# rkansal47/MPGAN

Measured on AMD Instinct MI355X. Metric: jets/sec (G+D step) MPGAN gluon N=30 bs=256 @1/2/4/8 MI355X, higher is better.
Workload: dtype split-16-bit MFMA, fp32 accumulate, fp32 in/out: f16 hi/lo x3 terms (forward), f16 x2 / x1 terms in per-sender dithered units (edge backward: data / weight gradients), bf16 hi/lo x3 (node network gradients); 1 GPU; MPGAN gluon-like jets (--jets g: lr_disc 3e-05, lr_gen 1e-05), N=30 particles, B=256 per GPU, one train_D+train_G iteration (LSGAN, RMSprop, D dropout 0.5); jets=g, loss=ls, fwd_two_term=False, global_batch=256, particles=30, multiplicity=gluon, parallelism=dp1, hip_graphs=True, graph_collectives=False

## Files before the change

include/mpgan_amd.h:

```cpp
#ifndef MPGAN_AMD_H
#define MPGAN_AMD_H
#include <stdint.h>
#ifdef __cplusplus
extern "C" {
#endif

typedef struct MpgGemm {
    const float* A;
    const float* A2;
    int lda, lda2, K1;
    const float* B;
    int ldb;
    float* C;
    int ldc;
    int M, N, K;
    long long split_stride;
    const float* bias;
    float out_scale;
    int act;
    float alpha;
    const uint64_t* seed;
    uint32_t drop_tag, drop_thr; float drop_scale;
    const float* gateH;
    int ldh, gate_act;
// ... 200 lines not shown
} MpgAttnDD;
int mpg_attn_dd(const MpgAttnDD* p, void* stream);

int mpg_rank_mask(const float* x, int ld_jet, int ld_part, const float* labels, int ld_lab, int B, int N,
                  float* mask, float* ignore, void* stream);

int mpg_jet_order(const float* mask, int B, int N, int* order, void* stream);

int mpg_gen_tail_fwd(const float* y, int ldy, const float* mask, float* out, int ldo, int V, int F, int act, void* stream);
int mpg_gen_tail_bwd(const float* dout, int ldd, const float* out, int ldo, float* dy, int ldy, int V, int F, int act,
                     void* stream);

typedef struct MpgDiscHead {
    const float* y; int ldy;
    const float* mask;
    const float* w; const float* bias;
    int B, N, F;
    int mean;
    int sigmoid;
    const uint64_t* seed; uint32_t tag, thr; float dscale;
    float* out;
    float* pooled; float* aux;
    int loss, gen_step, n_real; float inv_count;
    const float* gout;
    float* terms; float* loss_out;
    float* dy; int ld_dy;
    float* dw; float* db; int accumulate;
    const float* targets;
    const float* loss_extra;
} MpgDiscHead;
int mpg_disc_head_fwd(const MpgDiscHead* p, void* stream);
int mpg_disc_head_bwd(const MpgDiscHead* p, void* stream);
int mpg_disc_head_loss(const MpgDiscHead* p, void* stream);

typedef struct MpgDiscHeadDD {
    const float* y; int ldy;
    const float* mask;
    const float* w; const float* bias;
    int B, N, F, mean, sigmoid;
    const uint64_t* seed; uint32_t tag, thr; float dscale;
    int mode;
    const float* g;
    const float* U; int ldu;
    const float* mu;
    float* gy; int ld_gy;
    float* gm;
    float* gg;
    float* part;
    float* gw; float* gb;
} MpgDiscHeadDD;
int mpg_disc_head_dd(const MpgDiscHeadDD* p, void* stream);

typedef struct MpgBridge {
    const float* x; int ldx;
    const float* W1; const float* b1;
    int act1;
    float* feat; int ldf;
    int M, row0, K, F, E;
    const float* W2; const float* b2;
    int act2; float alpha;
    const uint64_t* seed; uint32_t tag, thr; float dscale;
    float* e; int lde;
} MpgBridge;
typedef struct MpgBridgeBwd {
    const float* ge; int ldge;
    const float* e; int lde;
// ... 191 lines not shown
```

mpgan_amd/_lib.py:

```python
from __future__ import annotations

import ctypes as C
import glob
import os
import subprocess

_HERE = os.path.dirname(os.path.abspath(__file__))
CSRC = os.path.join(_HERE, "csrc")
LIBDIR = os.environ.get("MPG_LIBDIR") or os.path.join(_HERE, "lib")
LIBPATH = os.path.join(LIBDIR, "libmpgan_amd.so")
INCLUDE = os.path.join(os.path.dirname(_HERE), "include")

_u64p = C.POINTER(C.c_uint64)
_fp = C.c_void_p


class MpgGemm(C.Structure):
    _fields_ = [
        ("A", _fp), ("A2", _fp), ("lda", C.c_int), ("lda2", C.c_int), ("K1", C.c_int),
        ("B", _fp), ("ldb", C.c_int),
        ("C", _fp), ("ldc", C.c_int),
        ("M", C.c_int), ("N", C.c_int), ("K", C.c_int),
        ("split_stride", C.c_longlong),
        ("bias", _fp), ("out_scale", C.c_float), ("act", C.c_int), ("alpha", C.c_float),
# ... 260 lines not shown
    "mpg_gemm_wgrad_group": (C.c_int, [C.POINTER(MpgGemm), C.POINTER(C.c_int), C.c_int, C.c_void_p]),
    "mpg_splitk_reduce_group": (C.c_int, [C.POINTER(MpgReduceJob), C.c_int, C.c_void_p]),
    "mpg_splitk_reduce_group_dw": (C.c_int, [C.POINTER(MpgReduceJob), C.c_int, C.POINTER(MpgEdgeDw), C.c_void_p]),
    "mpg_slab_sums": (C.c_int, [_fp, C.c_int, C.c_uint64, _fp, C.c_int, C.c_uint64, _fp, C.c_int, C.c_int, C.c_void_p]),
    "mpg_gate": (C.c_int, [_fp, C.c_int, _fp, C.c_int, _fp, C.c_int, C.c_int, C.c_int, C.c_int, C.c_float,
                           _fp, C.c_uint32, C.c_uint32, C.c_float, C.c_void_p]),
    "mpg_dropout_mask": (C.c_int, [_fp, C.c_uint64, C.c_int, _fp, C.c_uint32, C.c_uint32, C.c_void_p]),
    "mpg_pack_weights": (C.c_int, [_fp, C.c_int, C.c_int, C.c_int, C.c_int, C.c_float, C.c_int, _fp, C.c_void_p]),
    "mpg_pack_many": (C.c_int, [C.POINTER(MpgPackJob), C.c_int, C.c_void_p]),
    "mpg_chain": (C.c_int, [C.POINTER(MpgChain), C.c_void_p]),
    "mpg_chain_route": (C.c_int, [C.POINTER(MpgChain)]),
    "mpg_edge_fwd": (C.c_int, [C.POINTER(MpgEdgeFwd), C.c_void_p]),
    "mpg_edge_fwd_fn": (C.c_int, [C.POINTER(MpgEdgeFwd), C.POINTER(MpgChain), C.POINTER(MpgChain), C.c_void_p]),
    "mpg_edge_bwd": (C.c_int, [C.POINTER(MpgEdgeBwd), C.c_void_p]),
    "mpg_edge_bwd_fn": (C.c_int, [C.POINTER(MpgEdgeBwd), C.POINTER(MpgChain), C.POINTER(MpgChain), C.c_void_p]),
    "mpg_edge_dw": (C.c_int, [C.POINTER(MpgEdgeDw), C.c_void_p]),
    "mpg_attn_fwd": (C.c_int, [C.POINTER(MpgAttn), C.c_void_p]),
    "mpg_attn_bwd": (C.c_int, [C.POINTER(MpgAttn), C.c_void_p]),
    "mpg_attn_dd": (C.c_int, [C.POINTER(MpgAttnDD), C.c_void_p]),
    "mpg_mab_fwd": (C.c_int, [C.POINTER(MpgMab), C.c_void_p]),
    "mpg_mab_bwd": (C.c_int, [C.POINTER(MpgMab), C.c_void_p]),
    "mpg_mab_chain_fwd": (C.c_int, [C.POINTER(MpgMabChain), C.c_void_p]),
    "mpg_knn_edge_fwd": (C.c_int, [C.POINTER(MpgKnnEdgeFwd), C.c_void_p]),
    "mpg_knn_edge_bwd": (C.c_int, [C.POINTER(MpgKnnEdgeBwd), C.c_void_p]),
    "mpg_knn_edge_jvp": (C.c_int, [C.POINTER(MpgKnnEdgeJvp), C.c_void_p]),
    "mpg_knn_sets": (C.c_int, [_fp, C.c_int, _fp, C.c_int, C.c_int, C.c_int, C.c_int, C.c_int, _fp, C.c_void_p]),
    "mpg_rank_mask": (C.c_int, [_fp, C.c_int, C.c_int, _fp, C.c_int, C.c_int, C.c_int, _fp, _fp, C.c_void_p]),
    "mpg_jet_order": (C.c_int, [_fp, C.c_int, C.c_int, _fp, C.c_void_p]),
    "mpg_gen_tail_fwd": (C.c_int, [_fp, C.c_int, _fp, _fp, C.c_int, C.c_int, C.c_int, C.c_int, C.c_void_p]),
    "mpg_gen_tail_bwd": (C.c_int, [_fp, C.c_int, _fp, C.c_int, _fp, C.c_int, C.c_int, C.c_int, C.c_int, C.c_void_p]),
    "mpg_disc_head_fwd": (C.c_int, [C.POINTER(MpgDiscHead), C.c_void_p]),
    "mpg_disc_head_bwd": (C.c_int, [C.POINTER(MpgDiscHead), C.c_void_p]),
    "mpg_disc_head_loss": (C.c_int, [C.POINTER(MpgDiscHead), C.c_void_p]),
    "mpg_disc_head_dd": (C.c_int, [C.POINTER(MpgDiscHeadDD), C.c_void_p]),
    "mpg_layernorm_fwd": (C.c_int, [_fp, C.c_int, _fp, _fp, _fp, C.c_int, _fp, C.c_int, C.c_int, C.c_float, C.c_void_p]),
    "mpg_layernorm_bwd": (C.c_int, [_fp, C.c_int, _fp, C.c_int, _fp, _fp, _fp, C.c_int, _fp, C.c_int, _fp, _fp, C.c_int,
                                    C.c_int, C.c_int, C.c_void_p]),
    "mpg_batchnorm_stats": (C.c_int, [_fp, C.c_int, C.c_int, C.c_int, _fp, C.c_int, _fp, _fp, C.c_void_p]),
    "mpg_batchnorm_apply": (C.c_int, [_fp, C.c_int, _fp, _fp, _fp, _fp, C.c_float, _fp, C.c_int, C.c_int, C.c_int, C.c_void_p]),
    "mpg_batchnorm_bwd": (C.c_int, [_fp, C.c_int, _fp, C.c_int, _fp, _fp, _fp, C.c_float, _fp, C.c_int, _fp, _fp, C.c_int, _fp, _fp,
                                    C.c_int, C.c_int, C.c_int, C.c_void_p]),
    "mpg_rmsprop": (C.c_int, [_fp, _fp, _fp, C.c_uint64, C.c_float, C.c_float, C.c_float, C.c_float, C.c_int, _fp, C.c_uint64, C.c_void_p]),
    "mpg_adam": (C.c_int, [_fp, _fp, _fp, _fp, _fp, C.c_uint64, C.c_float, C.c_float, C.c_float, C.c_float, C.c_float,
                           C.c_float, C.c_int, _fp, C.c_uint64, C.c_void_p]),
    "mpg_adadelta": (C.c_int, [_fp, _fp, _fp, _fp, C.c_uint64, C.c_float, C.c_float, C.c_float, C.c_float, C.c_int, _fp, C.c_uint64,
                               C.c_void_p]),
    "mpg_rmsprop_ema": (C.c_int, [_fp, _fp, _fp, C.c_uint64, C.c_float, C.c_float, C.c_float, C.c_float, C.c_int, _fp, C.c_uint64,
                                  C.POINTER(MpgEma), C.c_void_p]),
    "mpg_adam_ema": (C.c_int, [_fp, _fp, _fp, _fp, _fp, C.c_uint64, C.c_float, C.c_float, C.c_float, C.c_float, C.c_float,
                               C.c_float, C.c_int, _fp, C.c_uint64, C.POINTER(MpgEma), C.c_void_p]),
    "mpg_adadelta_ema": (C.c_int, [_fp, _fp, _fp, _fp, C.c_uint64, C.c_float, C.c_float, C.c_float, C.c_float, C.c_int, _fp, C.c_uint64,
                                   C.POINTER(MpgEma), C.c_void_p]),
    "mpg_ema_update_host": (C.c_int, [_fp, _fp, C.c_uint64, C.c_uint32, C.c_float, C.c_int, C.c_int]),
    "mpg_step_control": (C.c_int, [_fp, C.c_uint64, C.c_float, C.POINTER(MpgStepCtl), C.c_void_p]),
    "mpg_step_control_host": (C.c_int, [_fp, C.c_uint64, C.c_float, C.POINTER(MpgStepCtl)]),
    "mpg_rmsprop_ctl": (C.c_int, [_fp, _fp, _fp, C.c_uint64, C.c_float, C.c_float, C.c_float, C.c_float, C.c_int, _fp, C.c_uint64,
                                  C.POINTER(MpgStepCtl), C.POINTER(MpgEma), C.c_void_p]),
    "mpg_adam_ctl": (C.c_int, [_fp, _fp, _fp, _fp, _fp, C.c_uint64, C.c_float, C.c_float, C.c_float, C.c_float, C.c_float,
                               C.c_float, C.c_int, _fp, C.c_uint64, C.POINTER(MpgStepCtl), C.POINTER(MpgEma), C.c_void_p]),
    "mpg_adadelta_ctl": (C.c_int, [_fp, _fp, _fp, _fp, C.c_uint64, C.c_float, C.c_float, C.c_float, C.c_float, C.c_int, _fp, C.c_uint64,
                                   C.POINTER(MpgStepCtl), C.POINTER(MpgEma), C.c_void_p]),
    "mpg_bridge_fwd": (C.c_int, [C.POINTER(MpgBridge), C.c_void_p]),
    "mpg_bridge_bwd": (C.c_int, [C.POINTER(MpgBridgeBwd), C.c_void_p]),
    "mpg_normal": (C.c_int, [_fp, C.c_uint64, _fp, C.c_uint32, C.c_float, C.c_float, C.c_void_p]),
    "mpg_normal_rank_mask": (C.c_int, [_fp, C.c_int, C.c_int, C.c_int, _fp, C.c_uint32, C.c_float, C.c_float, _fp, C.c_int, _fp, _fp,
                                       C.c_void_p]),
# ... 213 lines not shown
```

mpgan_amd/csrc/head.hip:

```cpp
#include "common.h"
#include "../../include/mpgan_amd.h"

namespace {

__global__ __launch_bounds__(256) void rank_mask_kernel(const float* __restrict__ x, int ld_jet, int ld_part,
                                                        const float* __restrict__ labels, int ld_lab, int N,
                                                        float* __restrict__ mask, float* __restrict__ ignore) {
    extern __shared__ float xs[];
    const int b = blockIdx.x;
    for (int i = threadIdx.x; i < N; i += blockDim.x) xs[i] = x[(size_t)b * ld_jet + (size_t)i * ld_part];
    __syncthreads();
    const int n_minus_1 = (int)(labels[(size_t)b * ld_lab] * (float)N) - 1;
    for (int i = threadIdx.x; i < N; i += blockDim.x) {
        const float xi = xs[i];
        int rank = 0;
        for (int j = 0; j < N; ++j) {
            const float xj = xs[j];
            rank += (xj < xi) || (xj == xi && j < i);
        }
        mask[(size_t)b * N + i] = rank <= n_minus_1 ? 1.f : 0.f;
        if (ignore != nullptr) ignore[(size_t)b * N + i] = rank <= n_minus_1 ? 0.f : 1.f;
    }
}

__global__ __launch_bounds__(1024) void jet_order_kernel(const float* __restrict__ mask, int B, int N, int* __restrict__ order) {
    extern __shared__ int jo[];
    int* keys = jo;
    int* hist = jo + B;
    int* wcnt = jo + B + N + 2;
    const int nw = (B + 63) / 64, lane = threadIdx.x & 63;
    for (int t = threadIdx.x; t < N + 2; t += blockDim.x) hist[t] = 0;
    for (int t = threadIdx.x; t < nw * (N + 1); t += blockDim.x) wcnt[t] = 0;
    __syncthreads();
// ... 18 lines not shown
    for (int b0 = (threadIdx.x >> 6) * 64; b0 < B; b0 += blockDim.x) {
        const int b = b0 + lane;
        const int k = b < B ? keys[b] : -1;
        int below = 0;
        for (int l = 0; l < 64; ++l) {
            const int kl = __shfl(k, l, 64);
            below += (l < lane && kl == k);
        }
        if (b < B) order[hist[k] + wcnt[(b >> 6) * (N + 1) + k] + below] = b;
    }
}

__global__ __launch_bounds__(256) void gen_tail_fwd_kernel(const float* __restrict__ y, int ldy, const float* __restrict__ mask,
                                                           float* __restrict__ out, int ldo, int V, int F, int act) {
    const int v = blockIdx.x * blockDim.x + threadIdx.x;
    if (v >= V) return;
    for (int f = 0; f < F; ++f) {
        const float t = y[(size_t)v * ldy + f];
        out[(size_t)v * ldo + f] = act == 1 ? tanhf(t) : (act == 2 ? 1.f / (1.f + expf(-t)) : t);
    }
    if (mask != nullptr) out[(size_t)v * ldo + F] = mask[v] - 0.5f;
}

__global__ __launch_bounds__(256) void gen_tail_bwd_kernel(const float* __restrict__ dout, int ldd, const float* __restrict__ out, int ldo,
                                                           float* __restrict__ dy, int ldy, int V, int F, int act) {
    const int v = blockIdx.x * blockDim.x + threadIdx.x;
    if (v >= V) return;
    for (int f = 0; f < F; ++f) {
        const float o = out[(size_t)v * ldo + f], g = dout[(size_t)v * ldd + f];
        dy[(size_t)v * ldy + f] = act == 1 ? g * (1.f - o * o) : (act == 2 ? g * o * (1.f - o) : g);
    }
}

MPG_DEV float wave_sum(float x) {
#pragma unroll
    for (int o = 32; o > 0; o >>= 1) x += __shfl_xor(x, o, 64);
    return x;
}

MPG_DEV void disc_head_bwd_jet(const MpgDiscHead& p, const int b, const int lane, const float out, const float aux0);

template <bool FUSED>
__global__ __launch_bounds__(256) void disc_head_fwd_kernel(const MpgDiscHead p) {
    const int lane = threadIdx.x & 63, b = blockIdx.x * 4 + (threadIdx.x >> 6);
    if (b >= p.B) return;
    const float* yb = p.y + (size_t)b * p.N * p.ldy;
    float z = 0.f, msum = 0.f;
    for (int f0 = 0; f0 < p.F; f0 += 32) {
        const int f = f0 + (lane & 31);
        float a0 = 0.f, a1 = 0.f, a2 = 0.f, a3 = 0.f;
        auto term = [&](int i) {
            return i < p.N ? (p.mask ? p.mask[(size_t)b * p.N + i] : 1.f) * yb[(size_t)i * p.ldy + f] : 0.f;
        };
        if (f < p.F)
            for (int i = lane >> 5; i < p.N; i += 8) { a0 += term(i); a1 += term(i + 2); a2 += term(i + 4); a3 += term(i + 6); }
        float acc = (a0 + a1) + (a2 + a3);
        acc += __shfl_xor(acc, 32, 64);
        if (p.pooled != nullptr && lane < 32 && f < p.F) p.pooled[(size_t)b * p.F + f] = acc;
        z += (lane < 32 && f < p.F) ? acc * p.w[f] : 0.f;
    }
    if (p.mean) {
        for (int i = lane; i < p.N; i += 64) msum += p.mask ? p.mask[(size_t)b * p.N + i] : 1.f;
        msum = wave_sum(msum);
    }
    z = wave_sum(z);
    const float pool_scale = p.mean ? 1.f / (p.mask ? msum + 1e-12f : (float)p.N) : 1.f;
    z = z * pool_scale + (p.bias ? p.bias[0] : 0.f);
    float keep = 1.f;
    if (p.thr) {
        const uint64_t sd = *p.seed;
        keep = drop_keep_f((uint32_t)sd, (uint32_t)(sd >> 32), p.tag, (uint32_t)b, 0, p.thr) ? p.dscale : 0.f;
    }
    z *= keep;
    const float out = p.sigmoid ? 1.f / (1.f + expf(-z)) : z;
    if (lane == 0) {
        p.out[b] = out;
        if (p.aux != nullptr) { p.aux[2 * b] = keep * pool_scale; p.aux[2 * b + 1] = 0.f; }
    }
    if (FUSED) disc_head_bwd_jet(p, b, lane, out, keep * pool_scale);
}

MPG_DEV float loss_grad(int loss, float out, float t, float& term) {
    switch (loss) {
    case 0: term = (out - t) * (out - t); return 2.f * (out - t);
    case 1: {
        const float l1 = fmaxf(logf(out), -100.f), l0 = fmaxf(logf(1.f - out), -100.f);
        term = -(t * l1 + (1.f - t) * l0);
        return (out - t) / fmaxf((1.f - out) * out, 1e-12f);
    }
    case 2: term = t > 0.5f ? -out : out; return t > 0.5f ? -1.f : 1.f;
    default: {
        const float s = t > 0.5f ? -1.f : 1.f, m = 1.f + s * out;
        term = fmaxf(m, 0.f);
        return m > 0.f ? s : 0.f;
    }
    }
}

MPG_DEV void disc_head_bwd_jet(const MpgDiscHead& p, const int b, const int lane, const float out, const float aux0) {
    float g;
    if (p.loss >= 0) {
        const float t = p.targets != nullptr ? p.targets[b] : (b < p.n_real ? 1.f : 0.f);
        float term;
        g = loss_grad((p.gen_step && p.loss == 3) ? 2 : p.loss, out, t, term) * p.inv_count;
        if (lane == 0) p.terms[b] = term * p.inv_count;
    } else {
        g = p.gout[b];
    }
    const float gz = g * (p.sigmoid ? out * (1.f - out) : 1.f);
    const float gp = gz * aux0;
    if (lane == 0) p.aux[2 * b + 1] = gz * (aux0 != 0.f ? (p.thr ? p.dscale : 1.f) : 0.f);
    if (p.dy == nullptr) return;
    float* db_ = p.dy + (size_t)b * p.N * p.ld_dy;
    for (int f0 = 0; f0 < p.F; f0 += 32) {
        const int f = f0 + (lane & 31);
        if (f >= p.F) continue;
        const float wf = p.w[f] * gp;
        for (int i = lane >> 5; i < p.N; i += 2) db_[(size_t)i * p.ld_dy + f] = (p.mask ? p.mask[(size_t)b * p.N + i] : 1.f) * wf;
    }
}

__global__ __launch_bounds__(256) void disc_head_bwd_kernel(const MpgDiscHead p) {
    const int lane = threadIdx.x & 63, b = blockIdx.x * 4 + (threadIdx.x >> 6);
    if (b >= p.B) return;
    disc_head_bwd_jet(p, b, lane, p.out[b], p.aux[2 * b]);
}

__global__ __launch_bounds__(256) void disc_head_reduce_kernel(const MpgDiscHead p) {
    __shared__ float red[256];
    const int tid = threadIdx.x;
    if (blockIdx.x == 0) {
        if (p.loss >= 0 && p.loss_out != nullptr) {
            float s = 0.f;
            for (int b = tid; b < p.B; b += 256) s += p.terms[b];
            red[tid] = s;
            __syncthreads();
            for (int o = 128; o > 0; o >>= 1) { if (tid < o) red[tid] += red[tid + o]; __syncthreads(); }
            if (tid == 0) {
                float v = red[0];
                if (p.loss_extra != nullptr) v += *p.loss_extra;
                *p.loss_out = v;
            }
        }
        return;
    }
    if (p.dw == nullptr) return;
    const int f = (blockIdx.x - 1) * 4 + (tid >> 6), lane = tid & 63;
    if (f > p.F) return;
    const float ds = p.thr ? p.dscale : 1.f;
    auto term = [&](int b) {
        if (b >= p.B) return 0.f;
        const float gzp = p.aux[2 * b + 1];
// ... 267 lines not shown
}

extern "C" int mpg_gen_tail_fwd(const float* y, int ldy, const float* mask, float* out, int ldo, int V, int F, int act,
                                void* stream) {
    if (V <= 0 || F <= 0) return -1;
    hipLaunchKernelGGL(gen_tail_fwd_kernel, dim3((V + 255) / 256), dim3(256), 0, (hipStream_t)stream, y, ldy, mask, out, ldo, V, F, act);
    return (int)hipGetLastError();
}

extern "C" int mpg_gen_tail_bwd(const float* dout, int ldd, const float* out, int ldo, float* dy, int ldy, int V, int F,
                                int act, void* stream) {
    if (V <= 0 || F <= 0) return -1;
    hipLaunchKernelGGL(gen_tail_bwd_kernel, dim3((V + 255) / 256), dim3(256), 0, (hipStream_t)stream, dout, ldd, out, ldo, dy, ldy, V, F, act);
    return (int)hipGetLastError();
}

extern "C" int mpg_disc_head_fwd(const MpgDiscHead* p, void* stream) {
    if (p->B <= 0 || p->N <= 0 || p->F <= 0 || p->out == nullptr || p->aux == nullptr) return -1;
    hipLaunchKernelGGL(disc_head_fwd_kernel<false>, dim3((p->B + 3) / 4), dim3(256), 0, (hipStream_t)stream, *p);
    return (int)hipGetLastError();
}

extern "C" int mpg_disc_head_loss(const MpgDiscHead* p, void* stream) {
    if (p->B <= 0 || p->N <= 0 || p->F <= 0 || p->out == nullptr || p->aux == nullptr) return -1;
    if (p->loss < 0 || p->terms == nullptr) return -2;
    if (p->dw != nullptr && p->pooled == nullptr) return -2;
    hipStream_t st = (hipStream_t)stream;
    hipLaunchKernelGGL(disc_head_fwd_kernel<true>, dim3((p->B + 3) / 4), dim3(256), 0, st, *p);
    if (p->loss_out != nullptr || p->dw != nullptr)
        hipLaunchKernelGGL(disc_head_reduce_kernel, dim3(1 + (p->dw != nullptr ? (p->F + 1 + 3) / 4 : 0)), dim3(256), 0, st, *p);
    return (int)hipGetLastError();
}

extern "C" int mpg_disc_head_dd(const MpgDiscHeadDD* p, void* stream) {
    if (p->B <= 0 || p->N <= 0 || p->N > 1024 || p->F <= 0 || p->mode < 0 || p->mode > 1) return -1;
    if (p->y == nullptr || p->w == nullptr || (p->thr != 0 && p->seed == nullptr) || (p->mode == 1 && p->g == nullptr)) return -2;
    if ((p->gw != nullptr || p->gb != nullptr) && p->part == nullptr) return -2;
    if (p->gm != nullptr && p->mask == nullptr) return -2;
    if (p->ldy < p->F || (p->gy != nullptr && p->ld_gy < p->F) || (p->U != nullptr && p->ldu < p->F)) return -5;
    hipStream_t st = (hipStream_t)stream;
    hipLaunchKernelGGL(disc_head_dd_kernel, dim3(p->B), dim3(64), 8 * p->N * sizeof(float), st, *p);
    if (p->gw != nullptr || p->gb != nullptr)
        hipLaunchKernelGGL(disc_head_dd_reduce_kernel, dim3((p->F + 1 + 3) / 4), dim3(256), 0, st, p->part, p->B, p->F, p->gw, p->gb);
    return (int)hipGetLastError();
}

extern "C" int mpg_disc_head_bwd(const MpgDiscHead* p, void* stream) {
    if (p->B <= 0 || p->N <= 0 || p->F <= 0 || p->out == nullptr || p->aux == nullptr) return -1;
    if (p->loss >= 0 ? p->terms == nullptr : p->gout == nullptr) return -2;
    if (p->dw != nullptr && p->pooled == nullptr) return -2;
    hipStream_t st = (hipStream_t)stream;
    hipLaunchKernelGGL(disc_head_bwd_kernel, dim3((p->B + 3) / 4), dim3(256), 0, st, *p);
    if ((p->loss >= 0 && p->loss_out != nullptr) || p->dw != nullptr)
        hipLaunchKernelGGL(disc_head_reduce_kernel, dim3(1 + (p->dw != nullptr ? (p->F + 1 + 3) / 4 : 0)), dim3(256), 0, st, *p);
    return (int)hipGetLastError();
}
```

mpgan_amd/ops.py:

```python
from __future__ import annotations

import contextlib
import ctypes as C
import itertools
import os
import sys
import threading
from collections import namedtuple
from typing import Optional

import torch
from torch.autograd.function import once_differentiable

from . import _lib
from ._lib import MpgGemm, MpgEdgeFwd, MpgEdgeBwd, MpgEdgeDw, MpgKnnEdgeFwd, MpgKnnEdgeBwd, MpgKnnEdgeJvp, MpgPackJob, MpgChain, MpgReduceJob, check

H1, H2, H3 = 96, 160, 192
SC_W2, SC_W3 = 16.0, 64.0
SC_WN, SC_ACT = 64.0, 8.0
TAG_E0, TAG_E1, TAG_E2, TAG_N0, TAG_N1, TAG_N2, TAG_GENERIC = 1, 2, 3, 4, 5, 6, 7

OPTIONS = {
    "skip_masked": True,
    "lpt_order": True,
# ... 2733 lines not shown
        B, N, F = y.shape
        dev = y.device
        out = torch.empty((B,), device=dev, dtype=torch.float32)
        pooled = torch.empty((B, F), device=dev, dtype=torch.float32)
        aux = torch.empty((2 * B,), device=dev, dtype=torch.float32)
        tag = next_tag(dev, "head", drop_params(p_drop)[0] if training else 0) + TAG_GENERIC
        wv = w.reshape(-1)
        h = _head_struct(y, m, wv, b, mean, sigmoid, p_drop, training, tag, out, pooled, aux)
        check(_lib.lib().mpg_disc_head_fwd(C.byref(h), _stream()), "mpg_disc_head_fwd")
        ctx.save_for_backward(y, m, w, b, out, pooled, aux)
        ctx.cfg = (mean, sigmoid, p_drop, training, tag)
        return out

    @staticmethod
    @once_differentiable
    def backward(ctx, gout):
        y, m, w, b, out, pooled, aux = ctx.saved_tensors
        mean, sigmoid, p_drop, training, tag = ctx.cfg
        B, N, F = y.shape
        dev = y.device
        h = _head_struct(y, m, w.reshape(-1), b, mean, sigmoid, p_drop, training, tag, out, pooled, aux)
        gout = gout.contiguous()
        h.gout = _p(gout)
        dy = torch.empty((B, N, F), device=dev, dtype=torch.float32) if ctx.needs_input_grad[0] else None
        h.dy, h.ld_dy = _p(dy), F
        need_w = ctx.needs_input_grad[2]
        pg = ParamGrads(dev_state(dev), (w, b), (need_w, need_w and b is not None))
        (tw, tb), h.accumulate = pg.written(lambda: (torch.empty_like(w), None if b is None else torch.empty_like(b)))
        h.dw, h.db = _p(tw), _p(tb)
        check(_lib.lib().mpg_disc_head_bwd(C.byref(h), _stream()), "mpg_disc_head_bwd")
        return dy, None, *pg.slots(), None, None, None, None


def disc_head_loss(y, mask, w, b, *, mean, sigmoid, p_drop, training, loss, n_real, gen_step, count, loss_out,
                   want_dy=True, wgrad=None, targets=None, loss_extra=None):
    y, m = _head_inputs(y, mask)
    B, N, F = y.shape
    dev = y.device
    out = torch.empty((B,), device=dev, dtype=torch.float32)
    pooled = torch.empty((B, F), device=dev, dtype=torch.float32)
    aux = torch.empty((2 * B,), device=dev, dtype=torch.float32)
    terms = torch.empty((B,), device=dev, dtype=torch.float32)
    tag = next_tag(dev, "head", drop_params(p_drop)[0] if training else 0) + TAG_GENERIC
    h = _head_struct(y, m, w.reshape(-1), b, mean, sigmoid, p_drop, training, tag, out, pooled, aux)
    h.loss, h.gen_step, h.n_real, h.inv_count = LOSS_CODES[loss], int(gen_step), n_real, 1.0 / count
    h.terms, h.loss_out = _p(terms), _p(loss_out)
    dy = torch.empty((B, N, F), device=dev, dtype=torch.float32) if want_dy else None
    h.dy, h.ld_dy = _p(dy), F
    if wgrad is not None:
        h.dw, h.db, h.accumulate = _p(wgrad[0]), _p(wgrad[1]), 1
    for t, k, name in ((targets, B, "targets"), (loss_extra, 1, "loss_extra")):
        if t is not None:
            _chk(t, name)
            if not t.is_contiguous() or t.numel() != k or t.device != dev:
                raise ValueError(f"disc_head_loss: {name} must be contiguous with {k} elements on {dev}, got {tuple(t.shape)} on {t.device}")
    h.targets, h.loss_extra = _p(targets), _p(loss_extra)
    check(_lib.lib().mpg_disc_head_loss(C.byref(h), _stream()), "mpg_disc_head_loss")
    return out, dy


DiscHeadDDSettings = namedtuple("DiscHeadDDSettings", "mean sigmoid p_drop training keep param_grads", defaults=(0.0, True, None, True))
DD_HEAD_MAX_N = 1024


def gp_head_route(N: int, double_backward: bool, options=None) -> bool:
    opt = OPTIONS if options is None else options
    return bool(opt.get("gp_chain") and double_backward and 1 <= N <= DD_HEAD_MAX_N)


class _HeadState:
    __slots__ = ("cpu", "B", "N", "F", "mean", "sigmoid", "thr", "dscale", "tag", "seed_t", "kappa", "param_grads", "mask_shape",
                 "w_shape", "has_bias")


def _head_dd_terms(st, y, m, wv, b):
    t = y @ wv
    S = (t if m is None else m * t).sum(1)
    if not st.mean:
        d = torch.ones_like(S)
    elif m is None:
        d = torch.full_like(S, float(st.N))
    else:
        d = m.sum(1) + 1e-12
    c = S / d if (st.mean and m is not None) else torch.zeros_like(S)
    z = S / d + (0 if b is None else b.reshape(()))
    if st.kappa is not None:
        z = st.kappa * z
    if st.sigmoid:
        o = torch.sigmoid(z)
# ... 240 lines not shown
```

mpgan_amd/train.py:

```python
from __future__ import annotations

import copy
import ctypes as C
import os
from typing import Optional

import torch
from torch import nn

from . import _lib, ops, dist as mdist
from .mpgan import MPGenerator, MPDiscriminator
from .step_options import (ADA_DEFAULTS, AUG_SITES, AdaController, Augment, Augmenter, DeviceWords, Ema, EmaState, GradClip,
                           LabelDraw, LrSchedule, Schedule, SeedState, StepControl, ada_rule, effective_targets)

LR = {
    "g": (3e-5, 1e-5), "t": (6e-5, 2e-5), "q": (1.5e-5, 0.5e-5),
}


def default_mpgan(num_particles: int = 30, disc_dropout: float = 0.5, gen_dropout: float = 0.0, device="cuda",
                  loss: str = "ls", spectral_norm_gen: bool = False, spectral_norm_disc: bool = False,
                  batch_norm_gen: bool = False, batch_norm_disc: bool = False):
    def lin(p, bn=False, sn=False):
        return {"leaky_relu_alpha": 0.2, "dropout_p": p, "batch_norm": bn, "spectral_norm": sn}
# ... 299 lines not shown
        jets, self.jets = self.jets, None
        return jets


class TrainStep:

    def __init__(self, G: nn.Module, D: nn.Module, batch_size: int, num_particles: int, latent: int = 32,
                 lr_disc: float = 3e-5, lr_gen: float = 1e-5, noise_std: float = 0.2, use_graphs: bool = True,
                 process_group=None, world_size: int = 1, batch_real_fake: bool = True, loss: str = "ls",
                 optimizer: str = "rmsprop", betas=(0.9, 0.999), gp_lambda: float = 0.0,
                 graph_collectives: Optional[bool] = None, augment=None, loader=None, num_critic: int = 1, num_gen: int = 1,
                 track_epoch_losses: bool = False, label_smoothing: bool = False, label_noise: float = 0.0,
                 ema: Optional[Ema] = None, lr_schedule=None, grad_clip=None, gp_rows: Optional[bool] = None,
                 gp_attn: Optional[bool] = None, gp_chain: Optional[bool] = None, _ada_split: bool = False):
        if loss not in LOSSES:
            raise ValueError(f"loss must be one of {LOSSES}, got {loss!r}")
        self.dev = dev = next(G.parameters()).device
        gpu = dev.type == "cuda"
        self._labels = LabelDraw.from_args(loss, label_smoothing, label_noise, batch_size, dev)
        self.label_smoothing, self.label_noise, self.labels_on = bool(label_smoothing), float(label_noise), self._labels is not None
        if self.labels_on:
            self.label_targets, self.label_extra, self.label_drawn = self._labels.targets, self._labels.extra, self._labels.drawn
        for name, v in (("num_critic", num_critic), ("num_gen", num_gen)):
            if isinstance(v, bool) or not isinstance(v, int) or v < 1:
                raise ValueError(f"{name} must be an integer >= 1, got {v!r}")
        if num_critic > 1 and num_gen > 1:
            raise ValueError(f"num_critic = {num_critic} with num_gen = {num_gen}: the reference's --num-gen says \"num-critic must be "
                             "1 for this to apply\" (setup_training.py:249; train.py:841 ignores num_gen when num_critic > 1)")
        self.num_critic, self.num_gen = num_critic, num_gen
        self.last_ran = ()

        def _switch(name: str, default: str = "1") -> str:
            return os.environ.get(name, default)
        on = {k: _switch(k) != "0" for k in ("MPG_PARTS", "MPG_GEN_AHEAD", "MPG_GEN_AHEAD_LATE", "MPG_WGRAD_SIDE", "MPG_BRIDGE", "MPG_NOISE_MASK")}
        if graph_collectives is None:
            graph_collectives = _switch("MPG_GRAPH_COLLECTIVES", "") == "1"
        self.split_graphs = bool(_switch("MPG_SPLIT_GRAPHS", ""))
        self.gp_lambda = float(gp_lambda)
        self.gp_rows = bool(ops.OPTIONS["gp_rows"]) if gp_rows is None else bool(gp_rows)
        self.gp_attn = bool(ops.OPTIONS["gp_attn"]) if gp_attn is None else bool(gp_attn)
        self.gp_chain = bool(ops.OPTIONS["gp_chain"]) if gp_chain is None else bool(gp_chain)
        self.GP = torch.zeros((), device=dev)
        self.fixed_alpha = None
        self.G, self.D = G, D
        self.loss = loss
        self.batch_real_fake = batch_real_fake and not any(isinstance(m, nn.modules.batchnorm._BatchNorm) for m in D.modules())
        self.B, self.N, self.latent = batch_size, num_particles, latent
        self.lr_disc, self.lr_gen, self.noise_std = lr_disc, lr_gen, noise_std
        self.pg, self.world = process_group, world_size
        self.graph_collectives = bool(graph_collectives) and process_group is not None
        self.state = ops.dev_state(dev)
        if ema is not None and not isinstance(ema, Ema):
            raise TypeError(f"ema must be a step_options.Ema, got {type(ema).__name__}")
        def _pair(v, name, cls):
            pair = tuple(v) if isinstance(v, (tuple, list)) else (v, v)
            if len(pair) != 2 or not all(x is None or isinstance(x, cls) for x in pair):
                raise TypeError(f"{name} must be a step_options.{cls.__name__}, None or a (disc, gen) pair of those, got {v!r}")
            return pair
        scheds, clips = _pair(lr_schedule, "lr_schedule", LrSchedule), _pair(grad_clip, "grad_clip", GradClip)
        if not gpu and any(x is not None for x in scheds + clips):
            raise ValueError("lr_schedule / grad_clip: the step control is a launch in front of the fused optimizer launch; the "
                             "step's networks are not on a GPU")
        ctl_D, ctl_G = (None if s is None and c is None else StepControl(lr, s, c, dev)
                        for lr, s, c in zip((lr_disc, lr_gen), scheds, clips))
        self.fG = FlatParams(G, optimizer, betas, ema=ema, batch_size=batch_size * world_size, control=ctl_G)
        self._ema_twin = None
        ada_split = (augment is not None and AdaController.splits(augment, process_group, world_size, _ada_split)
# ... 18 lines not shown
        self._labels2 = torch.zeros(2 * batch_size, 1, device=dev)
        self._x3 = torch.zeros(2 * batch_size, num_particles, 3, device=dev)
        self._mask2 = torch.zeros(2 * batch_size, num_particles, 1, device=dev)
        self._ign2 = torch.zeros(2 * batch_size, num_particles, device=dev)
        self.parts = (gpu and hasattr(G, "generate_parts") and hasattr(D, "features_parts") and D.parts_ok()
                      and getattr(G, "use_mask", True) and not getattr(G, "lfc", False)
                      and getattr(G, "mask_args", {}).get("mask_c", True) and on["MPG_PARTS"])
        self.D_loss = torch.zeros((), device=dev)
        self.G_loss = torch.zeros((), device=dev)
        self.use_graphs = use_graphs and gpu
        self._graphs = None
        self._alone_graphs = {}
        self._pool = None
        self.epoch_sums = {k: torch.zeros((), device=dev) for k in ("D", "gp", "G")} if track_epoch_losses else None
        self._epoch_steps = 0
        self.gen_ahead = gpu and isinstance(G, MPGenerator) and _forward_writes_no_state(G) and on["MPG_GEN_AHEAD"]
        self._ahead = _GenAhead(dev)
        self.wgrad_side = gpu and on["MPG_WGRAD_SIDE"]
        if self.gp_lambda and (self.gp_rows or self.gp_chain):
            self.wgrad_side = False
        self._wside = None
        self.gen_ahead_late = self.gen_ahead and self.wgrad_side and on["MPG_GEN_AHEAD_LATE"]
        self.bridge = gpu and on["MPG_BRIDGE"]
        self.aug = self.aug_p = self._ada = None
        if augment is not None:
            self.aug_p = torch.full((1,), float(augment.aug_prob), device=dev)
            self.aug = Augmenter.from_args(augment, self.aug_p, batch_size)
        if self.aug is not None:
            self.aug_params = self.aug.params
            self._ada = AdaController.from_args(augment, self.aug_p, loss, batch_size, world_size, process_group, _ada_split,
                                                self.fD.tail)
        self.ada_state, self.ada_r = (None, None) if self._ada is None else (self._ada.state, self._ada.r)
        self.noise_mask = gpu and on["MPG_NOISE_MASK"]
        self.fixed_noise = None
        self._seen_versions = (self.fD.versions(), self.fG.versions())
        self._clean = {"D": True, "G": True}
        self.fG.carried = [c for c in (self._seed, self._schedule) if c is not None]
        self.fD.carried = [c for c in (self._ada,) if c is not None]
        if self.epoch_sums is not None:
            self.fG.carried.append(DeviceWords(self.epoch_sums.values()))
        if self.fG.ema_carried is not None:
            self.fG.carried.append(self.fG.ema_carried)
        for f in (self.fD, self.fG):
            if f.control is not None:
                f.carried.append(f.control)
        self.loader = None
        if loader is not None:
            self.attach_loader(loader)

    @property
    def gen_join(self):
        return self._ahead.joined

    def attach_loader(self, loader):
        if self._graphs is not None or self._alone_graphs:
            raise RuntimeError("attach_loader: the iteration has been captured already (the feed launch is part of the graph); "
                               "attach the loader before the first step")
        if loader.batch_size != self.B or loader.num_particles != self.N:
            raise ValueError(f"loader serves batches of {loader.batch_size} jets of {loader.num_particles} particles; the step "
                             f"was built for {self.B} x {self.N}")
        if loader.device != self.data.device:
            raise ValueError(f"loader lives on {loader.device}, the step on {self.data.device}")
        self.loader = loader
        self.fG.carried.append(DeviceWords([loader.cursor]))

    def _noise(self, which: int = 0):
# ... 85 lines not shown
                    fake, jets = None, (self.G.generate_rows(z, self.labels, premask=pm, **rows)[0], self._mask2, self._ign2)
                else:
                    fake, jets = self._x3[own], (self._x3, self._mask2, self._ign2)
                    self.G.generate_parts(z, self.labels, feat_out=fake, premask=pm, **rows)
            elif route == "into":
                fake, jets = self._dcat[own], self._dcat
                self.G.generate_into(self._noise(0), self.labels, fake)
            else:
                fake, jets = self.G(self._noise(0), self.labels), None
            if self.aug is not None:
                fake = self._augment(fake, AUG_SITES["D_fake"], in_place=True)
        return fake, jets

    def _generate(self, route: str):
        if route in ("rows", "parts"):
            z, pm = self._noise_masked(1)
            return (self.G.generate_rows if route == "rows" else self.G.generate_parts)(z, self.labels, premask=pm)
        return self.G(self._noise(1), self.labels)

    def _features(self, route: str, jets, labels, gen_step: bool):
        if route == "into":
            return self.D.features(jets, labels)
        x, mask, ign = jets
        if route == "parts":
            return self.D.features_parts(x, mask, labels, ignore=ign)
        head, real = self.G.bridge_head(), None
        if not gen_step:
            head, real = (head[0].detach(), None if head[1] is None else head[1].detach(), head[2]), self._x3
        return self.D.features_rows(x, head, real, mask, labels, ignore=ign)

    def _head_loss_backward(self, y, mask, gen_step: bool, then=None):
        w, b, mean, sigmoid, p = self.D.fused_head()
        lab = {"targets": self.label_targets, "loss_extra": self.label_extra} if self.labels_on and not gen_step else {}
        out, dy = ops.disc_head_loss(y, mask, w, b, mean=mean, sigmoid=sigmoid, p_drop=p, training=self.D.training, loss=self.loss,
                                     n_real=self.B, gen_step=gen_step, count=self.B, loss_out=self.G_loss if gen_step else self.D_loss,
                                     want_dy=True, wgrad=None if gen_step else (w.grad, None if b is None else b.grad), **lab)
        if self._ada is not None and not gen_step:
            self._ada.update(out, self.B)
        self._sum_epoch("G" if gen_step else "D")
        self._backward(y, dy, then)

    def _sum_epoch(self, key: str):
        if self.epoch_sums is not None:
            self.epoch_sums[key].add_({"D": self.D_loss, "gp": self.GP, "G": self.G_loss}[key])

    def _seg_D(self, join: bool = True, fork: bool = True):
        self._open_batch()
        if fork and self.gen_ahead and not self.gen_ahead_late:
            self._fork_generator()
        self.G.eval()
        if not self._clean["D"]:
            self.fD.zero_grad()
        self._clean["D"] = False
        _set_requires_grad(self.fD, True)
        try:
            self._seg_D_body(self._fork_generator if fork and self.gen_ahead_late else None)
        finally:
            if join:
                self._ahead.join("seg_D")

    def _open_batch(self):
        if self.loader is not None:
            self.loader.feed(self)
        self.state.grad_into_param = True
        self.state.order_cache = None
        self.D.train()

    def _close_batch(self, net: str):
        flat, lr = (self.fD, self.lr_disc) if net == "D" else (self.fG, self.lr_gen)
# ... 331 lines not shown
```

Measured before the change: 136,400 jets/s.

## Fuse discriminator head loss/backward into last MP layer's FN gradient chain kernel

Adds a head_chain kernel that computes the discriminator head forward, loss gradient and dy per jet, then feeds the result straight into the chained FN-gradient MFMA tiles of the last message-passing layer. It writes dy and the chain input in one pass. A separate reduce kernel handles loss and weight-gradient reductions. The aim is to remove a kernel launch and the global round-trip of dy between the head loss and the layer backward. The cost is that jets spanning tile boundaries are recomputed redundantly, and the kernel only applies under strict shape and config conditions.

```diff
diff --git a/include/mpgan_amd.h b/include/mpgan_amd.h
--- a/include/mpgan_amd.h
+++ b/include/mpgan_amd.h
@@ -256,6 +256,8 @@
 int mpg_disc_head_fwd(const MpgDiscHead* p, void* stream);
 int mpg_disc_head_bwd(const MpgDiscHead* p, void* stream);
 int mpg_disc_head_loss(const MpgDiscHead* p, void* stream);
+int mpg_disc_head_reduce(const MpgDiscHead* p, void* stream);
+int mpg_disc_head_chain(const MpgDiscHead* p, const MpgChain* c, int waves, void* stream);
 
 typedef struct MpgDiscHeadDD {
     const float* y; int ldy;
diff --git a/mpgan_amd/_lib.py b/mpgan_amd/_lib.py
--- a/mpgan_amd/_lib.py
+++ b/mpgan_amd/_lib.py
@@ -316,6 +316,8 @@
     "mpg_disc_head_fwd": (C.c_int, [C.POINTER(MpgDiscHead), C.c_void_p]),
     "mpg_disc_head_bwd": (C.c_int, [C.POINTER(MpgDiscHead), C.c_void_p]),
     "mpg_disc_head_loss": (C.c_int, [C.POINTER(MpgDiscHead), C.c_void_p]),
+    "mpg_disc_head_reduce": (C.c_int, [C.POINTER(MpgDiscHead), C.c_void_p]),
+    "mpg_disc_head_chain": (C.c_int, [C.POINTER(MpgDiscHead), C.POINTER(MpgChain), C.c_int, C.c_void_p]),
     "mpg_disc_head_dd": (C.c_int, [C.POINTER(MpgDiscHeadDD), C.c_void_p]),
     "mpg_layernorm_fwd": (C.c_int, [_fp, C.c_int, _fp, _fp, _fp, C.c_int, _fp, C.c_int, C.c_int, C.c_float, C.c_void_p]),
     "mpg_layernorm_bwd": (C.c_int, [_fp, C.c_int, _fp, C.c_int, _fp, _fp, _fp, C.c_int, _fp, C.c_int, _fp, _fp, C.c_int,
diff --git a/mpgan_amd/csrc/head.hip b/mpgan_amd/csrc/head.hip
--- a/mpgan_amd/csrc/head.hip
+++ b/mpgan_amd/csrc/head.hip
@@ -1,4 +1,5 @@
 #include "common.h"
+#include "head_impl.h"
 #include "../../include/mpgan_amd.h"
 
 namespace {
@@ -83,92 +84,13 @@
     }
 }
 
-MPG_DEV float wave_sum(float x) {
-#pragma unroll
-    for (int o = 32; o > 0; o >>= 1) x += __shfl_xor(x, o, 64);
-    return x;
-}
-
-MPG_DEV void disc_head_bwd_jet(const MpgDiscHead& p, const int b, const int lane, const float out, const float aux0);
-
 template <bool FUSED>
 __global__ __launch_bounds__(256) void disc_head_fwd_kernel(const MpgDiscHead p) {
     const int lane = threadIdx.x & 63, b = blockIdx.x * 4 + (threadIdx.x >> 6);
     if (b >= p.B) return;
-    const float* yb = p.y + (size_t)b * p.N * p.ldy;
-    float z = 0.f, msum = 0.f;
-    for (int f0 = 0; f0 < p.F; f0 += 32) {
-        const int f = f0 + (lane & 31);
-        float a0 = 0.f, a1 = 0.f, a2 = 0.f, a3 = 0.f;
-        auto term = [&](int i) {
-            return i < p.N ? (p.mask ? p.mask[(size_t)b * p.N + i] : 1.f) * yb[(size_t)i * p.ldy + f] : 0.f;
-        };
-        if (f < p.F)
-            for (int i = lane >> 5; i < p.N; i += 8) { a0 += term(i); a1 += term(i + 2); a2 += term(i + 4); a3 += term(i + 6); }
-        float acc = (a0 + a1) + (a2 + a3);
-        acc += __shfl_xor(acc, 32, 64);
-        if (p.pooled != nullptr && lane < 32 && f < p.F) p.pooled[(size_t)b * p.F + f] = acc;
-        z += (lane < 32 && f < p.F) ? acc * p.w[f] : 0.f;
-    }
-    if (p.mean) {
-        for (int i = lane; i < p.N; i += 64) msum += p.mask ? p.mask[(size_t)b * p.N + i] : 1.f;
-        msum = wave_sum(msum);
-    }
-    z = wave_sum(z);
-    const float pool_scale = p.mean ? 1.f / (p.mask ? msum + 1e-12f : (float)p.N) : 1.f;
-    z = z * pool_scale + (p.bias ? p.bias[0] : 0.f);
-    float keep = 1.f;
-    if (p.thr) {
-        const uint64_t sd = *p.seed;
-        keep = drop_keep_f((uint32_t)sd, (uint32_t)(sd >> 32), p.tag, (uint32_t)b, 0, p.thr) ? p.dscale : 0.f;
-    }
-    z *= keep;
-    const float out = p.sigmoid ? 1.f / (1.f + expf(-z)) : z;
-    if (lane == 0) {
-        p.out[b] = out;
-        if (p.aux != nullptr) { p.aux[2 * b] = keep * pool_scale; p.aux[2 * b + 1] = 0.f; }
-    }
-    if (FUSED) disc_head_bwd_jet(p, b, lane, out, keep * pool_scale);
-}
-
-MPG_DEV float loss_grad(int loss, float out, float t, float& term) {
-    switch (loss) {
-    case 0: term = (out - t) * (out - t); return 2.f * (out - t);
-    case 1: {
-        const float l1 = fmaxf(logf(out), -100.f), l0 = fmaxf(logf(1.f - out), -100.f);
-        term = -(t * l1 + (1.f - t) * l0);
-        return (out - t) / fmaxf((1.f - out) * out, 1e-12f);
-    }
-    case 2: term = t > 0.5f ? -out : out; return t > 0.5f ? -1.f : 1.f;
-    default: {
-        const float s = t > 0.5f ? -1.f : 1.f, m = 1.f + s * out;
-        term = fmaxf(m, 0.f);
-        return m > 0.f ? s : 0.f;
-    }
-    }
-}
-
-MPG_DEV void disc_head_bwd_jet(const MpgDiscHead& p, const int b, const int lane, const float out, const float aux0) {
-    float g;
-    if (p.loss >= 0) {
-        const float t = p.targets != nullptr ? p.targets[b] : (b < p.n_real ? 1.f : 0.f);
-        float term;
-        g = loss_grad((p.gen_step && p.loss == 3) ? 2 : p.loss, out, t, term) * p.inv_count;
-        if (lane == 0) p.terms[b] = term * p.inv_count;
-    } else {
-        g = p.gout[b];
-    }
-    const float gz = g * (p.sigmoid ? out * (1.f - out) : 1.f);
-    const float gp = gz * aux0;
-    if (lane == 0) p.aux[2 * b + 1] = gz * (aux0 != 0.f ? (p.thr ? p.dscale : 1.f) : 0.f);
-    if (p.dy == nullptr) return;
-    float* db_ = p.dy + (size_t)b * p.N * p.ld_dy;
-    for (int f0 = 0; f0 < p.F; f0 += 32) {
-        const int f = f0 + (lane & 31);
-        if (f >= p.F) continue;
-        const float wf = p.w[f] * gp;
-        for (int i = lane >> 5; i < p.N; i += 2) db_[(size_t)i * p.ld_dy + f] = (p.mask ? p.mask[(size_t)b * p.N + i] : 1.f) * wf;
-    }
+    float aux0;
+    const float out = disc_head_fwd_jet(p, b, lane, true, aux0);
+    if (FUSED) disc_head_bwd_jet(p, b, lane, out, aux0);
 }
 
 __global__ __launch_bounds__(256) void disc_head_bwd_kernel(const MpgDiscHead p) {
@@ -502,6 +424,15 @@
     return (int)hipGetLastError();
 }
 
+extern "C" int mpg_disc_head_reduce(const MpgDiscHead* p, void* stream) {
+    if (p->B <= 0 || p->F <= 0 || p->aux == nullptr) return -1;
+    if (p->loss >= 0 && p->loss_out != nullptr && p->terms == nullptr) return -2;
+    if (p->dw != nullptr && p->pooled == nullptr) return -2;
+    if (!(p->loss >= 0 && p->loss_out != nullptr) && p->dw == nullptr) return 0;
+    hipLaunchKernelGGL(disc_head_reduce_kernel, dim3(1 + (p->dw != nullptr ? (p->F + 1 + 3) / 4 : 0)), dim3(256), 0, (hipStream_t)stream, *p);
+    return (int)hipGetLastError();
+}
+
 extern "C" int mpg_disc_head_dd(const MpgDiscHeadDD* p, void* stream) {
     if (p->B <= 0 || p->N <= 0 || p->N > 1024 || p->F <= 0 || p->mode < 0 || p->mode > 1) return -1;
     if (p->y == nullptr || p->w == nullptr || (p->thr != 0 && p->seed == nullptr) || (p->mode == 1 && p->g == nullptr)) return -2;
diff --git a/mpgan_amd/csrc/head_chain.hip b/mpgan_amd/csrc/head_chain.hip
--- /dev/null
+++ b/mpgan_amd/csrc/head_chain.hip
@@ -0,0 +1,139 @@
+#include "chain2_impl.h"
+#include "chain_int.h"
+#include "head_impl.h"
+
+namespace {
+
+template <int DROP, int NW, typename FT, typename BR, typename BS>
+MPG_DEV void hc_stage(const MpgDiscHead& h, const MpgChain& p, const int m0, char* fb0, char* scratch, FT&& first_tile, BR&& bias_request,
+                      BS&& bias_store, const uint32_t seed_lo, const uint32_t seed_hi, const float ascale) {
+    typedef typename FragT<false>::type V;
+    using I0 = std::integral_constant<int, 0>;
+    using I1 = std::integral_constant<int, 1>;
+    constexpr int KS0 = 2;
+    const int tid = threadIdx.x, lane = tid & 63;
+    const int w = __builtin_amdgcn_readfirstlane(tid >> 6);
+    const int N = h.N, F = h.F, M = p.M;
+    const int b0 = m0 / N, b1 = min(m0 + 31, M - 1) / N;
+    float* sgp = reinterpret_cast<float*>(scratch);
+    const int u = min(tid, KS0 * 64 - 1), rr = u >> 2, ks = (u >> 1) & 1, hh = u & 1;
+    const int mm = m0 + rr, mc = min(mm, M - 1);
+    const float mi = h.mask != nullptr ? h.mask[mc] : 1.f;
+    float w8[8];
+#pragma unroll
+    for (int k = 0; k < 8; ++k) w8[k] = h.w[min(16 * ks + 8 * (k >> 2) + 4 * hh + (k & 3), F - 1)];
+    first_tile(I0{});
+    bias_request();
+    for (int j = w; j <= b1 - b0; j += NW) {
+        const int b = b0 + j;
+        const bool own = b * N >= m0;
+        float aux0;
+        const float out = disc_head_fwd_jet(h, b, lane, own, aux0);
+        const float gp = disc_head_grad_jet(h, b, lane, out, aux0, own);
+        if (lane == 0) sgp[j] = gp;
+    }
+    __syncthreads();
+    if (tid < KS0 * 64) {
+        V* fb = reinterpret_cast<V*>(fb0);
+        const int K = p.L[0].K;
+        const bool live = mm < M;
+        const float gp = sgp[mc / N - b0];
+        const uint32_t in_thr = p.in_thr;
+        const bool in_on = in_thr != 0u;
+        const float in_s = in_on ? p.in_scale : 1.f;
+        const __amdgpu_buffer_rsrc_t rio = __builtin_amdgcn_make_buffer_rsrc(
+            p.in_out, 0, p.in_out != nullptr ? (int)((size_t)M * p.ld_in_out * 4) : 0, 0x00020000);
+        const __amdgpu_buffer_rsrc_t rdy = __builtin_amdgcn_make_buffer_rsrc(
+            h.dy, 0, h.dy != nullptr ? (int)((size_t)M * h.ld_dy * 4) : 0, 0x00020000);
+        float v[8];
+#pragma unroll
+        for (int half = 0; half < 2; ++half) {
+            const int f = 16 * ks + 8 * half + 4 * hh;
+            float x4[4], d4[4];
+            uint32_t wd = 0;
+            if constexpr (DROP == 2) wd = drop_word(seed_lo, seed_hi, p.in_tag, (uint32_t)mm, DROP_BIT_GRP + (uint32_t)(f >> 5)) >> (f & 31);
+            if constexpr (DROP == 1) wd = drop_word(seed_lo, seed_hi, p.in_tag, (uint32_t)mm, (uint32_t)(f >> 2));
+#pragma unroll
+            for (int e = 0; e < 4; ++e) {
+                const float wf = w8[4 * half + e] * gp;
+                d4[e] = mi * wf;
+                float xv = (live && f + e < K) ? d4[e] : 0.f;
+                if constexpr (DROP != 0) {
+                    const bool keep = (DROP == 2 ? ((wd >> e) & 1u) != 0u : drop_keep(wd, e, in_thr)) || !in_on;
+                    xv = keep ? xv * in_s : 0.f;
+                }
+                x4[e] = xv;
+                v[4 * half + e] = xv * ascale;
+            }
+            const bool st = live && f + 4 <= K;
+            __builtin_amdgcn_raw_buffer_store_b128(
+                c2_u32x4{__builtin_bit_cast(uint32_t, d4[0]), __builtin_bit_cast(uint32_t, d4[1]), __builtin_bit_cast(uint32_t, d4[2]),
+                         __builtin_bit_cast(uint32_t, d4[3])},
+                rdy, st ? (int)(((size_t)mm * h.ld_dy + f) * 4) : -1, 0, 0);
+            __builtin_amdgcn_raw_buffer_store_b128(
+                c2_u32x4{__builtin_bit_cast(uint32_t, x4[0]), __builtin_bit_cast(uint32_t, x4[1]), __builtin_bit_cast(uint32_t, x4[2]),
+                         __builtin_bit_cast(uint32_t, x4[3])},
+                rio, st ? (int)(((size_t)mm * p.ld_in_out + f) * 4) : -1, 0, 0);
+        }
+        V hi, lo;
+        split8(v, hi, lo);
+        const int ln = rr + 32 * hh;
+        fb[(ks * 2 + 0) * 64 + ln] = hi;
+        fb[(ks * 2 + 1) * 64 + ln] = lo;
+    }
+    first_tile(I1{});
+    bias_store();
+}
+
+template <int DROP, int NW>
+__global__ __launch_bounds__(64 * NW, 1) void head_chain_kernel(const MpgDiscHead h, const MpgChain p) {
+    extern __shared__ __attribute__((aligned(16))) char smem[];
+    const int m0 = blockIdx.x * 32;
+    auto stage = [&](auto&& first_tile, auto&& bias_request, auto&& bias_store, const uint32_t seed_lo, const uint32_t seed_hi,
+                     const float ascale) {
+        hc_stage<DROP, NW>(h, p, m0, smem, smem + C2_FB, first_tile, bias_request, bias_store, seed_lo, seed_hi, ascale);
+    };
+    c2_body<false, 2, 16, 16, DROP, 3, 0, false, NW>(p, m0, 32, smem, smem + C2_FB, reinterpret_cast<float*>(smem + 2 * C2_FB), stage);
+}
+
+template <int DROP, int NW>
+int hc_launch(const MpgDiscHead* h, const MpgChain* c, hipStream_t st) {
+    return mpg_go<head_chain_kernel<DROP, NW>>(dim3((c->M + 31) / 32), dim3(64 * NW), C2_LDS, st, *h, *c);
+}
+template <int NW>
+int hc_launch_drop(const MpgDiscHead* h, const MpgChain* c, int drop, hipStream_t st) {
+    if (drop == 2) return hc_launch<2, NW>(h, c, st);
+    if (drop == 1) return hc_launch<1, NW>(h, c, st);
+    return hc_launch<0, NW>(h, c, st);
+}
+
+int hc_waves(int rows) {
+    (void)rows;
+    return 8;
+}
+
+}
+
+extern "C" int mpg_disc_head_chain(const MpgDiscHead* p, const MpgChain* c, int waves, void* stream) {
+    if (p->B <= 0 || p->N <= 0 || p->F <= 0 || p->out == nullptr || p->aux == nullptr || p->y == nullptr || p->w == nullptr) return -1;
+    if (c->M <= 0 || c->nlayers < 1 || c->nlayers > 3) return -1;
+    if (waves != 0 && waves != 4 && waves != 8) return -1;
+    if (p->dw != nullptr && p->pooled == nullptr) return -2;
+    if (p->thr != 0 && p->seed == nullptr) return -2;
+    if (!(c->alpha >= 0.f && c->alpha <= 1.f)) return -4;
+    if (p->loss < 0 || p->loss > 3 || p->terms == nullptr) return MPG_FN_NA;
+    if (p->N < 2 || p->F > 32 || p->F % 4 != 0 || p->ldy < p->F) return MPG_FN_NA;
+    if ((size_t)p->B * p->N != (size_t)c->M || c->f16) return MPG_FN_NA;
+    if (c->nlayers != 3 || c->a_slabs != 1 || c->K1 != c->L[0].K || c->L[0].K != p->F) return MPG_FN_NA;
+    for (int l = 0; l < 2; ++l)
+        if (c->L[l].N > 256 || c->L[l + 1].K != c->L[l].N) return MPG_FN_NA;
+    if (c->in_out != nullptr && (c->ld_in_out % 4 != 0 || c->ld_in_out < p->F || ((uintptr_t)c->in_out & 15) != 0)) return MPG_FN_NA;
+    if (p->dy != nullptr && (p->ld_dy % 4 != 0 || p->ld_dy < p->F || ((uintptr_t)p->dy & 15) != 0 ||
+                             (size_t)c->M * p->ld_dy * 4 >= 0x7fffffffull)) return MPG_FN_NA;
+    if (c->in_thr != 0 && c->seed == nullptr) return MPG_FN_NA;
+    MpgChain2Plan plan;
+    if (mpg_chain2_decide(c, &plan) == MPG_CHAIN2_NA || plan.shape != C2_FN_GRAD || plan.sl) return MPG_FN_NA;
+    const int nw = waves ? waves : hc_waves(c->M);
+    hipStream_t st = (hipStream_t)stream;
+    return nw == 8 ? hc_launch_drop<8>(p, c, plan.drop, st) : hc_launch_drop<4>(p, c, plan.drop, st);
+}
diff --git a/mpgan_amd/csrc/head_impl.h b/mpgan_amd/csrc/head_impl.h
--- /dev/null
+++ b/mpgan_amd/csrc/head_impl.h
@@ -0,0 +1,96 @@
+#pragma once
+#include "common.h"
+#include "../../include/mpgan_amd.h"
+
+namespace {
+
+MPG_DEV float wave_sum(float x) {
+#pragma unroll
+    for (int o = 32; o > 0; o >>= 1) x += __shfl_xor(x, o, 64);
+    return x;
+}
+
+MPG_DEV float disc_head_fwd_jet(const MpgDiscHead& p, const int b, const int lane, const bool own, float& aux0) {
+    const float* yb = p.y + (size_t)b * p.N * p.ldy;
+    float z = 0.f, msum = 0.f;
+    for (int f0 = 0; f0 < p.F; f0 += 32) {
+        const int f = f0 + (lane & 31);
+        float a0 = 0.f, a1 = 0.f, a2 = 0.f, a3 = 0.f;
+        auto term = [&](int i) {
+            return i < p.N ? (p.mask ? p.mask[(size_t)b * p.N + i] : 1.f) * yb[(size_t)i * p.ldy + f] : 0.f;
+        };
+        if (f < p.F)
+            for (int i = lane >> 5; i < p.N; i += 8) { a0 += term(i); a1 += term(i + 2); a2 += term(i + 4); a3 += term(i + 6); }
+        float acc = (a0 + a1) + (a2 + a3);
+        acc += __shfl_xor(acc, 32, 64);
+        if (own && p.pooled != nullptr && lane < 32 && f < p.F) p.pooled[(size_t)b * p.F + f] = acc;
+        z += (lane < 32 && f < p.F) ? acc * p.w[f] : 0.f;
+    }
+    if (p.mean) {
+        for (int i = lane; i < p.N; i += 64) msum += p.mask ? p.mask[(size_t)b * p.N + i] : 1.f;
+        msum = wave_sum(msum);
+    }
+    z = wave_sum(z);
+    const float pool_scale = p.mean ? 1.f / (p.mask ? msum + 1e-12f : (float)p.N) : 1.f;
+    z = z * pool_scale + (p.bias ? p.bias[0] : 0.f);
+    float keep = 1.f;
+    if (p.thr) {
+        const uint64_t sd = *p.seed;
+        keep = drop_keep_f((uint32_t)sd, (uint32_t)(sd >> 32), p.tag, (uint32_t)b, 0, p.thr) ? p.dscale : 0.f;
+    }
+    z *= keep;
+    const float out = p.sigmoid ? 1.f / (1.f + expf(-z)) : z;
+    aux0 = keep * pool_scale;
+    if (own && lane == 0) {
+        p.out[b] = out;
+        if (p.aux != nullptr) { p.aux[2 * b] = aux0; p.aux[2 * b + 1] = 0.f; }
+    }
+    return out;
+}
+
+MPG_DEV float loss_grad(int loss, float out, float t, float& term) {
+    switch (loss) {
+    case 0: term = (out - t) * (out - t); return 2.f * (out - t);
+    case 1: {
+        const float l1 = fmaxf(logf(out), -100.f), l0 = fmaxf(logf(1.f - out), -100.f);
+        term = -(t * l1 + (1.f - t) * l0);
+        return (out - t) / fmaxf((1.f - out) * out, 1e-12f);
+    }
+    case 2: term = t > 0.5f ? -out : out; return t > 0.5f ? -1.f : 1.f;
+    default: {
+        const float s = t > 0.5f ? -1.f : 1.f, m = 1.f + s * out;
+        term = fmaxf(m, 0.f);
+        return m > 0.f ? s : 0.f;
+    }
+    }
+}
+
+MPG_DEV float disc_head_grad_jet(const MpgDiscHead& p, const int b, const int lane, const float out, const float aux0, const bool own) {
+    float g;
+    if (p.loss >= 0) {
+        const float t = p.targets != nullptr ? p.targets[b] : (b < p.n_real ? 1.f : 0.f);
+        float term;
+        g = loss_grad((p.gen_step && p.loss == 3) ? 2 : p.loss, out, t, term) * p.inv_count;
+        if (own && lane == 0) p.terms[b] = term * p.inv_count;
+    } else {
+        g = p.gout[b];
+    }
+    const float gz = g * (p.sigmoid ? out * (1.f - out) : 1.f);
+    const float gp = gz * aux0;
+    if (own && lane == 0) p.aux[2 * b + 1] = gz * (aux0 != 0.f ? (p.thr ? p.dscale : 1.f) : 0.f);
+    return gp;
+}
+
+MPG_DEV void disc_head_bwd_jet(const MpgDiscHead& p, const int b, const int lane, const float out, const float aux0) {
+    const float gp = disc_head_grad_jet(p, b, lane, out, aux0, true);
+    if (p.dy == nullptr) return;
+    float* db_ = p.dy + (size_t)b * p.N * p.ld_dy;
+    for (int f0 = 0; f0 < p.F; f0 += 32) {
+        const int f = f0 + (lane & 31);
+        if (f >= p.F) continue;
+        const float wf = p.w[f] * gp;
+        for (int i = lane >> 5; i < p.N; i += 2) db_[(size_t)i * p.ld_dy + f] = (p.mask ? p.mask[(size_t)b * p.N + i] : 1.f) * wf;
+    }
+}
+
+}
diff --git a/mpgan_amd/ops.py b/mpgan_amd/ops.py
--- a/mpgan_amd/ops.py
+++ b/mpgan_amd/ops.py
@@ -2789,8 +2789,38 @@
         return dy, None, *pg.slots(), None, None, None, None
 
 
+def head_chain_node(y):
+    node = y.grad_fn
+    if node is None or type(node).__name__ != "FusedMPLayerFnBackward" or getattr(node, "knn", None) is not None:
+        return None
+    if getattr(node, "cfg", None) is None or getattr(node, "packed", None) is None or not any(node.needs_input_grad):
+        return None
+    try:
+        sv = mplayer_saved(node)
+    except RuntimeError:
+        return None
+    cfg = node.cfg
+    if sv.h1 is None or sv.h2 is None or tuple(y.shape) != (cfg.B, cfg.N, sv.V3.shape[0]) or not y.is_contiguous():
+        return None
+    return node
+
+
+def _head_chain(h, dy, node, waves):
+    B, N, F = dy.shape
+    fng = _fn_grad_chain(node, dy.view(B * N, F))
+    if fng.dz3.data_ptr() != dy.data_ptr():
+        h.dy = None
+    rc = _lib.lib().mpg_disc_head_chain(C.byref(h), C.byref(fng.chain), waves, _stream())
+    if rc == _lib.MPG_FN_NA:
+        h.dy = _p(dy)
+        return False
+    check(rc, "mpg_disc_head_chain")
+    node.pre = FnGradsDone(fng, gy_ptr=dy.data_ptr(), keep=dy)
+    return True
+
+
 def disc_head_loss(y, mask, w, b, *, mean, sigmoid, p_drop, training, loss, n_real, gen_step, count, loss_out,
-                   want_dy=True, wgrad=None, targets=None, loss_extra=None):
+                   want_dy=True, wgrad=None, targets=None, loss_extra=None, chain_node=None, waves=0):
     y, m = _head_inputs(y, mask)
     B, N, F = y.shape
     dev = y.device
@@ -2812,6 +2842,9 @@
             if not t.is_contiguous() or t.numel() != k or t.device != dev:
                 raise ValueError(f"disc_head_loss: {name} must be contiguous with {k} elements on {dev}, got {tuple(t.shape)} on {t.device}")
     h.targets, h.loss_extra = _p(targets), _p(loss_extra)
+    if chain_node is not None and dy is not None and _head_chain(h, dy, chain_node, waves):
+        check(_lib.lib().mpg_disc_head_reduce(C.byref(h), _stream()), "mpg_disc_head_reduce")
+        return out, dy
     check(_lib.lib().mpg_disc_head_loss(C.byref(h), _stream()), "mpg_disc_head_loss")
     return out, dy
 
diff --git a/mpgan_amd/train.py b/mpgan_amd/train.py
--- a/mpgan_amd/train.py
+++ b/mpgan_amd/train.py
@@ -355,7 +355,8 @@
 
         def _switch(name: str, default: str = "1") -> str:
             return os.environ.get(name, default)
-        on = {k: _switch(k) != "0" for k in ("MPG_PARTS", "MPG_GEN_AHEAD", "MPG_GEN_AHEAD_LATE", "MPG_WGRAD_SIDE", "MPG_BRIDGE", "MPG_NOISE_MASK")}
+        on = {k: _switch(k) != "0" for k in ("MPG_PARTS", "MPG_GEN_AHEAD", "MPG_GEN_AHEAD_LATE", "MPG_WGRAD_SIDE", "MPG_BRIDGE", "MPG_NOISE_MASK",
+                                                 "MPG_HEAD_CHAIN")}
         if graph_collectives is None:
             graph_collectives = _switch("MPG_GRAPH_COLLECTIVES", "") == "1"
         self.split_graphs = bool(_switch("MPG_SPLIT_GRAPHS", ""))
@@ -440,6 +441,8 @@
                                                 self.fD.tail)
         self.ada_state, self.ada_r = (None, None) if self._ada is None else (self._ada.state, self._ada.r)
         self.noise_mask = gpu and on["MPG_NOISE_MASK"]
+        self.head_chain = gpu and on["MPG_HEAD_CHAIN"]
+        self.head_chain_waves = 0
         self.fixed_noise = None
         self._seen_versions = (self.fD.versions(), self.fG.versions())
         self._clean = {"D": True, "G": True}
@@ -591,9 +594,10 @@
     def _head_loss_backward(self, y, mask, gen_step: bool, then=None):
         w, b, mean, sigmoid, p = self.D.fused_head()
         lab = {"targets": self.label_targets, "loss_extra": self.label_extra} if self.labels_on and not gen_step else {}
+        fuse = {"chain_node": ops.head_chain_node(y), "waves": self.head_chain_waves} if self.head_chain else {}
         out, dy = ops.disc_head_loss(y, mask, w, b, mean=mean, sigmoid=sigmoid, p_drop=p, training=self.D.training, loss=self.loss,
                                      n_real=self.B, gen_step=gen_step, count=self.B, loss_out=self.G_loss if gen_step else self.D_loss,
-                                     want_dy=True, wgrad=None if gen_step else (w.grad, None if b is None else b.grad), **lab)
+                                     want_dy=True, wgrad=None if gen_step else (w.grad, None if b is None else b.grad), **lab, **fuse)
         if self._ada is not None and not gen_step:
             self._ada.update(out, self.B)
         self._sum_epoch("G" if gen_step else "D")
```

Measured after the change: 137,600 jets/s (median of 6 runs). About the same (+0.9%).
